# karfly/learnable-triangulation-pytorch

Measured on NVIDIA H100. Metric: volumetric samples/sec (4-view 384x384, 64^3 grid), higher is better.
Workload: dtype fp16x3 (split-fp16 operands, 3 wgmma products per term, fp32 accumulate)

## Files before the change

learnable-triangulation-pytorch_b200/csrc/conv_fold.cu:

```cuda
#include "tc_common.cuh"
#include "conv_tc_params.cuh"

namespace lt {

constexpr int kFoldThreads = 384;
constexpr int kFoldSmem = 227 * 1024;

template <int K>
struct FoldTile;
template <>
struct FoldTile<3> { static constexpr int BH = 8, BD = 2, KDS = 3; static constexpr bool RES = true; };
template <>
struct FoldTile<7> { static constexpr int BH = 16, BD = 2, KDS = 1; static constexpr bool RES = false; };

template <int K, int NC>
struct FoldCfg {
  static constexpr int BW = 8, BH = FoldTile<K>::BH, BD = FoldTile<K>::BD, KDS = FoldTile<K>::KDS;
  static constexpr bool RES = FoldTile<K>::RES;
  static constexpr int WBOX = BW + K - 1, HBOX = BH + K - 1, DBOX = BD + KDS - 1;
  static constexpr int A_BYTES = WBOX * HBOX * DBOX * 128;
  static constexpr int ASTAGES = K / KDS;
  static constexpr int TAP = NC * 128;
  static constexpr int B_SLICE = RES ? K * K * K * TAP : KDS * K * TAP;
  static constexpr int BLOCKS = BH * BD / 8;
  static constexpr int MB = RES ? BLOCKS : BLOCKS / 2;
  static constexpr int AVAIL = kFoldSmem - 1024 - 256;
  static constexpr int ARING_FIT = RES ? (AVAIL - B_SLICE) / A_BYTES : 2;
  static constexpr int ARING = ARING_FIT > 4 ? 4 : ARING_FIT;
  static constexpr int BRING_FIT = RES ? 1 : (AVAIL - ARING * A_BYTES) / B_SLICE;
  static constexpr int BRING = BRING_FIT > 4 ? 4 : BRING_FIT;
  static constexpr int A_OFF = BRING * B_SLICE;
  static constexpr int BAR_OFF = A_OFF + ARING * A_BYTES;
  static constexpr size_t SMEM = (size_t)BAR_OFF + 256 + 1024;
  static_assert(BW * BH * BD == (RES ? 128 : 256) && BH % 8 == 0 && MB == 2, "two m64 blocks of whole 8-wide lines per warpgroup");
  static_assert(A_BYTES % 1024 == 0 && B_SLICE % 1024 == 0, "boxes must start on 1024-byte swizzle atoms");
  static_assert(ARING >= 2 && BRING >= (RES ? 1 : 2) && 2 * (ARING + BRING) * 8 <= 256 && SMEM <= (size_t)kFoldSmem, "shared memory");
};

__device__ __forceinline__ void fold_tile_origin(const TcParams& p, int t, int& ow0, int& oh0, int& od0, int& nb) {
  ow0 = (t % p.tw) * p.bw; t /= p.tw;
  oh0 = (t % p.th) * p.bh; t /= p.th;
  od0 = (t % p.td) * p.bd;
  nb = t / p.td;
}

__device__ __forceinline__ void fold_load_line(uint32_t (&f)[2][4], uint32_t box, uint32_t row, uint32_t m) {
  const uint32_t a = box + row * 128u, sw = row & 7u;
  ldmatrix_x4(f[0], a + ((m ^ sw) << 4));
  ldmatrix_x4(f[1], a + (((m + 4u) ^ sw) << 4));
}

template <int NC>
__device__ __forceinline__ void fold_tap(float (&d1)[NC / 2], float (&d2)[NC / 2], const uint32_t (&l0)[2][4],
                                         const uint32_t (&l1)[2][4], uint64_t bd, uint32_t acc) {
  uint32_t a[4][4];
#pragma unroll
  for (int s = 0; s < 4; ++s) {
    const int q = s >> 1, c = 2 * (s & 1);
    a[s][0] = l0[q][c]; a[s][1] = l1[q][c]; a[s][2] = l0[q][c + 1]; a[s][3] = l1[q][c + 1];
  }
  wgmma_f16_rs<NC>(d1, a[0], bd, acc);
  wgmma_f16_rs<NC>(d1, a[1], bd + 2, 1u);
  wgmma_f16_rs<NC>(d2, a[0], bd + 4, acc);
  wgmma_f16_rs<NC>(d2, a[1], bd + 6, 1u);
  wgmma_f16_rs<NC>(d2, a[2], bd, 1u);
  wgmma_f16_rs<NC>(d2, a[3], bd + 2, 1u);
}

template <int K, int NC>
__global__ void __launch_bounds__(kFoldThreads, 1) conv_fold_kernel(const __grid_constant__ CUtensorMap tmA,
                                                                    const __grid_constant__ CUtensorMap tmB, const TcParams p) {
  using C = FoldCfg<K, NC>;
  extern __shared__ uint8_t smem_raw[];
  uint8_t* smem = reinterpret_cast<uint8_t*>((reinterpret_cast<uintptr_t>(smem_raw) + 1023) & ~(uintptr_t)1023);
  uint8_t* bsm = smem;
  uint8_t* asm_ = smem + C::A_OFF;
  uint64_t* afull = reinterpret_cast<uint64_t*>(smem + C::BAR_OFF);
  uint64_t* aempty = afull + C::ARING;
  uint64_t* bfull = aempty + C::ARING;
  uint64_t* bempty = bfull + C::BRING;

  const int wg = __shfl_sync(0xffffffffu, (int)(threadIdx.x >> 7), 0);
  const int lane = threadIdx.x & 31;
  const int ntiles = p.tw * p.th * p.td * p.tn;

  if (threadIdx.x == 0) {
    for (int s = 0; s < C::ARING; ++s) { mbar_init(&afull[s], 1); mbar_init(&aempty[s], C::RES ? 128 : 256); }
    for (int s = 0; s < C::BRING; ++s) { mbar_init(&bfull[s], 1); mbar_init(&bempty[s], 2); }
    fence_barrier_init();
    prefetch_tmap(&tmA);
    prefetch_tmap(&tmB);
  }
  __syncthreads();

  if (wg == 0) {
    regs_release_producer();
    if (threadIdx.x < 32) {
      if (C::RES && elect_one()) {
        mbar_expect_tx(&bfull[0], (uint32_t)C::B_SLICE);
        tma_load_3d(bsm, &tmB, &bfull[0], 0, 0, 0);
      }
      int sa = 0, sb = 0;
      uint32_t pa = 0, pb = 0;
      for (int t = blockIdx.x; t < ntiles; t += gridDim.x) {
        int ow0, oh0, od0, nb;
        fold_tile_origin(p, t, ow0, oh0, od0, nb);
        for (int as = 0; as < C::ASTAGES; ++as) {
          mbar_wait(&aempty[sa], pa ^ 1u);
          if (elect_one()) {
            mbar_expect_tx(&afull[sa], (uint32_t)C::A_BYTES);
            tma_load_5d(asm_ + (size_t)sa * C::A_BYTES, &tmA, &afull[sa], 0, ow0 - K / 2, oh0 - K / 2, od0 + as * C::KDS - K / 2, nb);
          }
          __syncwarp();
          if (++sa == C::ARING) { sa = 0; pa ^= 1u; }
          if constexpr (!C::RES) {
            for (int kw = 0; kw < K; ++kw) {
              mbar_wait(&bempty[sb], pb ^ 1u);
              if (elect_one()) {
                mbar_expect_tx(&bfull[sb], (uint32_t)C::B_SLICE);
                tma_load_3d(bsm + (size_t)sb * C::B_SLICE, &tmB, &bfull[sb], 0, 0, (kw * K + as * C::KDS) * K);
              }
              __syncwarp();
              if (++sb == C::BRING) { sb = 0; pb ^= 1u; }
            }
          }
        }
      }
    }
    return;
  }

  regs_claim_consumer();
  const int g = wg - 1, warp = (threadIdx.x >> 5) & 3;
  float d1[C::MB][NC / 2], d2[C::MB][NC / 2];
#pragma unroll
  for (int b = 0; b < C::MB; ++b)
#pragma unroll
    for (int i = 0; i < NC / 2; ++i) { d1[b][i] = 0.f; d2[b][i] = 0.f; }
  int blk_dd[C::MB], blk_hb[C::MB];
  uint32_t row0[C::MB];
#pragma unroll
  for (int b = 0; b < C::MB; ++b) {
    const int blk = C::RES ? b : C::MB * g + b;
    blk_dd[b] = blk / (C::BH / 8);
    blk_hb[b] = blk % (C::BH / 8);
    row0[b] = (uint32_t)((blk_dd[b] * C::HBOX + blk_hb[b] * 8 + 2 * warp) * C::WBOX + (lane & 7));
  }
  const uint32_t mlane = (uint32_t)(lane >> 3);
  const int r_lo = warp * 16 + (lane >> 2);
  const int c2 = 2 * (lane & 3);
  const uint32_t bsm0 = smem_u32(bsm), asm0 = smem_u32(asm_);
  const bool wg_lead = (threadIdx.x & 127) == 0;
  if (C::RES) mbar_wait(&bfull[0], 0);
  const int kt0 = C::RES ? g : 0, kstep = C::RES ? 2 : 1;
  int bprev = -1;
  for (int kt = kt0;; kt += kstep) {
    const int t = blockIdx.x + kt * gridDim.x;
    if (t >= ntiles) break;
#pragma unroll 1
    for (int as = 0; as < C::ASTAGES; ++as) {
      const int na = kt * C::ASTAGES + as;
      const int sa = na % C::ARING;
      mbar_wait(&afull[sa], (uint32_t)(na / C::ARING) & 1u);
      const uint32_t box = asm0 + (uint32_t)(sa * C::A_BYTES);
#pragma unroll 1
      for (int kw = 0; kw < K; ++kw) {
        const int nbs = na * K + kw;
        const int sb = C::RES ? 0 : nbs % C::BRING;
        if (!C::RES) mbar_wait(&bfull[sb], (uint32_t)(nbs / C::BRING) & 1u);
        const uint32_t bslice = bsm0 + (uint32_t)(sb * C::B_SLICE);
#pragma unroll
        for (int kdl = 0; kdl < C::KDS; ++kdl) {
          const int kd = as * C::KDS + kdl;
          const uint32_t roff = (uint32_t)(kdl * C::HBOX * C::WBOX + kw);
          uint32_t ln[K + 1][C::MB][2][4];
#pragma unroll
          for (int b = 0; b < C::MB; ++b) fold_load_line(ln[0][b], box, row0[b] + roff, mlane);
#pragma unroll
          for (int kh = 0; kh < K; ++kh) {
#pragma unroll
            for (int b = 0; b < C::MB; ++b) fold_load_line(ln[kh + 1][b], box, row0[b] + roff + (uint32_t)((kh + 1) * C::WBOX), mlane);
            wg_fence();
            const int tap = C::RES ? (kw * K + kd) * K + kh : kdl * K + kh;
            const uint64_t bd = make_sw128_desc(bslice + (uint32_t)(tap * C::TAP));
            const uint32_t acc = (as == 0 && kw == 0 && kdl == 0 && kh == 0) ? 0u : 1u;
#pragma unroll
            for (int b = 0; b < C::MB; ++b) fold_tap<NC>(d1[b], d2[b], ln[kh][b], ln[kh + 1][b], bd, acc);
            wg_commit();
            wg_wait<1>();
            if (!C::RES && kh == 0 && bprev >= 0) {
              if (wg_lead) mbar_arrive_local(&bempty[bprev]);
              bprev = -1;
            }
          }
        }
        if (!C::RES) bprev = sb;
      }
      mbar_arrive_local(&aempty[sa]);
    }
    wg_wait<0>();
    if (!C::RES) {
      if (wg_lead) mbar_arrive_local(&bempty[bprev]);
      bprev = -1;
    }
#pragma unroll
    for (int b = 0; b < C::MB; ++b) { wg_fence_regs(d1[b]); wg_fence_regs(d2[b]); }

    int ow0, oh0, od0, nb;
    fold_tile_origin(p, t, ow0, oh0, od0, nb);
#pragma unroll
    for (int b = 0; b < C::MB; ++b) {
#pragma unroll
      for (int h = 0; h < 2; ++h) {
        const int r = r_lo + 8 * h;
        const int ow = ow0 + (r & 7), oh = oh0 + blk_hb[b] * 8 + (r >> 3), od = od0 + blk_dd[b];
        if (!(ow < p.OW && oh < p.OH && od < p.OD)) continue;
        const long opix = (((long)nb * p.FD + od) * p.FH + oh) * p.FW + ow;
        conv_epilogue_row<NC>(p, d1[b], d2[b], h, opix, 0, c2);
        if constexpr (NC == 16) {
          const float z[8] = {0.f, 0.f, 0.f, 0.f, 0.f, 0.f, 0.f, 0.f};
          conv_epilogue_row<16>(p, z, z, h, opix, 16, c2);
        }
      }
    }
  }
}

template <int K, int NC>
static int launch_fold(const CUtensorMap& tmA, const CUtensorMap& tmB, const TcParams& p, cudaStream_t st) {
  using C = FoldCfg<K, NC>;
  static DeviceOnce configured;
  if (configured.first()) {
    cudaError_t e = cudaFuncSetAttribute(conv_fold_kernel<K, NC>, cudaFuncAttributeMaxDynamicSharedMemorySize, kFoldSmem);
    if (e != cudaSuccess) return fail(LT_ERR_CUDA, "conv_fold: cudaFuncSetAttribute: %s", cudaGetErrorString(e));
  }
  const long ntiles = (long)p.tw * p.th * p.td * p.tn;
  const int grid = (int)(ntiles < sm_count() ? ntiles : sm_count());
  conv_fold_kernel<K, NC><<<grid, kFoldThreads, C::SMEM, st>>>(tmA, tmB, p);
  cudaError_t e = cudaGetLastError();
  if (e != cudaSuccess) return fail(LT_ERR_CUDA, "conv_fold_kernel: %s", cudaGetErrorString(e));
  return LT_OK;
}

template <int K, int NC>
static int conv_fold_run(const lt_conv_desc* d, const void* in, const void* weight, const float* scale, const float* shift,
                         const void* residual, void* out, cudaStream_t st) {
  using C = FoldCfg<K, NC>;
  TcParams p;
  fill_params(d, p, 1, NC, NC, 3, scale, shift, residual, out);
  p.bw = C::BW; p.bh = C::BH; p.bd = C::BD; p.bn = 1;
  p.tw = ceil_div(d->OW, p.bw); p.th = ceil_div(d->OH, p.bh); p.td = ceil_div(d->OD, p.bd); p.tn = d->N;
  p.stages = C::ARING;
  CUtensorMap tmA, tmB;
  int rc = make_in_map(&tmA, d, C::WBOX, C::HBOX, C::DBOX, 1, in);
  if (rc) return rc;
  const uint64_t dims[3] = {64, (uint64_t)NC, (uint64_t)K * K * K};
  const uint64_t str[2] = {128, (uint64_t)NC * 128};
  const uint32_t bx[3] = {64, (uint32_t)NC, (uint32_t)(C::B_SLICE / C::TAP)};
  rc = make_map(&tmB, weight, 3, dims, str, bx, nullptr, 1);
  if (rc) return rc;
  return launch_fold<K, NC>(tmA, tmB, p, st);
}

int conv_fold_supported(const lt_conv_desc* d) {
  const bool cubic = d->KD == d->KH && d->KH == d->KW && (d->KW == 3 || d->KW == 7);
  const int pd = d->KW / 2;
  return cubic && d->Cin == 32 && d->Cout <= 32 && d->sd == 1 && d->sh == 1 && d->sw == 1 && d->pd == pd && d->ph == pd &&
         d->pw == pd && d->OD == d->ID && d->OH == d->IH && d->OW == d->IW && d->osd == 1 && d->osh == 1 && d->osw == 1 &&
         d->ood == 0 && d->ooh == 0 && d->oow == 0 && d->FD == d->OD && d->FH == d->OH && d->FW == d->OW && d->FC == 32 &&
         d->in_format == LT_FMT_S32 && d->IW >= 16;
}

int conv_fold_fwd(const lt_conv_desc* d, const void* in, const void* weight, const float* scale, const float* shift,
                  const void* residual, void* out, void* stream) {
  LT_REQUIRE(conv_fold_supported(d), "conv_fold: unsupported layer shape");
  const cudaStream_t st = (cudaStream_t)stream;
  const bool narrow = d->Cout <= 16;
  if (d->KW == 3)
    return narrow ? conv_fold_run<3, 16>(d, in, weight, scale, shift, residual, out, st)
                  : conv_fold_run<3, 32>(d, in, weight, scale, shift, residual, out, st);
  return narrow ? conv_fold_run<7, 16>(d, in, weight, scale, shift, residual, out, st)
                : conv_fold_run<7, 32>(d, in, weight, scale, shift, residual, out, st);
}

__global__ void __launch_bounds__(256) fold_pack_weights_kernel(const float* __restrict__ w, sh_t* __restrict__ out, int K, int Cout,
                                                                int NC) {
  const int total = K * K * K * NC * 32;
  for (int i = blockIdx.x * blockDim.x + threadIdx.x; i < total; i += gridDim.x * blockDim.x) {
    const int ci = i % 32;
    int r = i / 32;
    const int co = r % NC; r /= NC;
    const int kh = r % K; r /= K;
    const int kd = r % K;
    const int kw = r / K;
    const int tap = (kd * K + kh) * K + kw;
    const float v = co < Cout ? w[((long)tap * 32 + ci) * Cout + co] : 0.0f;
    sh_t hi, lo;
    split_s32(v, hi, lo);
    sh_t* rowp = out + ((long)((kw * K + kd) * K + kh) * NC + co) * 64;
    rowp[ci] = hi;
    rowp[32 + ci] = lo;
  }
}

}

using namespace lt;

extern "C" size_t lt_conv_fold_weight_bytes(int K, int Cout) {
  const int NC = (Cout + 15) & ~15;
  return (size_t)K * K * K * NC * 128;
}

extern "C" int lt_conv_fold_pack_weights(const float* w_tap_ci_co, void* packed, int K, int Cout, void* stream) {
  LT_REQUIRE(w_tap_ci_co && packed && (K == 3 || K == 7) && Cout > 0 && Cout <= 32, "conv_fold_pack_weights: bad arguments");
  const int NC = (Cout + 15) & ~15;
  const int total = K * K * K * NC * 32;
  fold_pack_weights_kernel<<<ceil_div(total, 256), 256, 0, (cudaStream_t)stream>>>(w_tap_ci_co, reinterpret_cast<sh_t*>(packed), K,
                                                                                   Cout, NC);
  LT_CHECK_LAUNCH("fold_pack_weights_kernel");
  return LT_OK;
}
```

learnable-triangulation-pytorch_b200/csrc/tc_common.cuh:

```cuda
#pragma once
#include "common.cuh"
#include <cuda.h>

namespace lt {

__device__ __forceinline__ uint32_t smem_u32(const void* p) { return (uint32_t)__cvta_generic_to_shared(p); }

__device__ __forceinline__ bool elect_one() {
  uint32_t pred;
  asm volatile("{\n\t.reg .pred p;\n\telect.sync _|p, 0xffffffff;\n\tselp.u32 %0, 1, 0, p;\n\t}" : "=r"(pred));
  return pred != 0;
}

__device__ __forceinline__ void mbar_init(uint64_t* bar, uint32_t count) {
  asm volatile("mbarrier.init.shared::cta.b64 [%0], %1;" ::"r"(smem_u32(bar)), "r"(count));
}
__device__ __forceinline__ void mbar_expect_tx(uint64_t* bar, uint32_t bytes) {
  asm volatile("mbarrier.arrive.expect_tx.shared::cta.b64 _, [%0], %1;" ::"r"(smem_u32(bar)), "r"(bytes) : "memory");
}
__device__ __forceinline__ bool mbar_try_wait(uint64_t* bar, uint32_t parity) {
  uint32_t ok;
  asm volatile(
      "{\n\t.reg .pred p;\n\t"
      "mbarrier.try_wait.parity.shared::cta.b64 p, [%1], %2;\n\t"
      "selp.u32 %0, 1, 0, p;\n\t}"
      : "=r"(ok)
      : "r"(smem_u32(bar)), "r"(parity)
      : "memory");
  return ok != 0;
}
__device__ __forceinline__ void mbar_wait(uint64_t* bar, uint32_t parity) {
  if (mbar_try_wait(bar, parity)) return;
  const long long t0 = clock64();
  while (!mbar_try_wait(bar, parity)) {
    if (clock64() - t0 > 4000000000LL) __trap();
  }
}
__device__ __forceinline__ void mbar_arrive_local(uint64_t* bar) {
  asm volatile("mbarrier.arrive.shared::cta.b64 _, [%0];" ::"r"(smem_u32(bar)) : "memory");
}
__device__ __forceinline__ void fence_barrier_init() { asm volatile("fence.mbarrier_init.release.cluster;" ::: "memory"); }
__device__ __forceinline__ void fence_proxy_async() { asm volatile("fence.proxy.async.shared::cta;" ::: "memory"); }

__device__ __forceinline__ void tma_load_5d(void* dst, const CUtensorMap* map, uint64_t* bar, int c0, int c1, int c2, int c3, int c4) {
  asm volatile(
      "cp.async.bulk.tensor.5d.shared::cluster.global.mbarrier::complete_tx::bytes [%0], [%1, {%3, %4, %5, %6, %7}], [%2];"
      ::"r"(smem_u32(dst)), "l"(map), "r"(smem_u32(bar)), "r"(c0), "r"(c1), "r"(c2), "r"(c3), "r"(c4)
      : "memory");
}
__device__ __forceinline__ void tma_load_3d(void* dst, const CUtensorMap* map, uint64_t* bar, int c0, int c1, int c2) {
  asm volatile(
      "cp.async.bulk.tensor.3d.shared::cluster.global.mbarrier::complete_tx::bytes [%0], [%1, {%3, %4, %5}], [%2];"
      ::"r"(smem_u32(dst)), "l"(map), "r"(smem_u32(bar)), "r"(c0), "r"(c1), "r"(c2)
      : "memory");
}
__device__ __forceinline__ void tma_load_2d(void* dst, const CUtensorMap* map, uint64_t* bar, int c0, int c1) {
  asm volatile(
      "cp.async.bulk.tensor.2d.shared::cluster.global.mbarrier::complete_tx::bytes [%0], [%1, {%3, %4}], [%2];"
      ::"r"(smem_u32(dst)), "l"(map), "r"(smem_u32(bar)), "r"(c0), "r"(c1)
      : "memory");
}
__device__ __forceinline__ void tma_store_5d(const CUtensorMap* map, const void* src, int c0, int c1, int c2, int c3, int c4) {
  asm volatile("cp.async.bulk.tensor.5d.global.shared::cta.bulk_group [%0, {%2, %3, %4, %5, %6}], [%1];"
               ::"l"(map), "r"(smem_u32(src)), "r"(c0), "r"(c1), "r"(c2), "r"(c3), "r"(c4)
               : "memory");
}
__device__ __forceinline__ void bulk_commit() { asm volatile("cp.async.bulk.commit_group;" ::: "memory"); }
__device__ __forceinline__ void bulk_wait_read0() { asm volatile("cp.async.bulk.wait_group.read 0;" ::: "memory"); }
__device__ __forceinline__ void bulk_wait0() { asm volatile("cp.async.bulk.wait_group 0;" ::: "memory"); }
__device__ __forceinline__ uint4 lds128(uint32_t a) {
  uint4 v;
  asm volatile("ld.shared.v4.u32 {%0, %1, %2, %3}, [%4];" : "=r"(v.x), "=r"(v.y), "=r"(v.z), "=r"(v.w) : "r"(a));
  return v;
}
__device__ __forceinline__ uint32_t lds32(uint32_t a) {
  uint32_t v;
  asm volatile("ld.shared.b32 %0, [%1];" : "=r"(v) : "r"(a));
  return v;
}
__device__ __forceinline__ void sts32(uint32_t a, uint32_t v) { asm volatile("st.shared.b32 [%0], %1;" ::"r"(a), "r"(v)); }
__device__ __forceinline__ float2 lds_f2(uint32_t a) {
  float2 v;
  asm volatile("ld.shared.v2.f32 {%0, %1}, [%2];" : "=f"(v.x), "=f"(v.y) : "r"(a));
  return v;
}
__device__ __forceinline__ void sts_f2(uint32_t a, float2 v) {
  asm volatile("st.shared.v2.f32 [%0], {%1, %2};" ::"r"(a), "f"(v.x), "f"(v.y));
}
__device__ __forceinline__ void prefetch_tmap(const CUtensorMap* map) {
  asm volatile("prefetch.tensormap [%0];" ::"l"(map) : "memory");
}

__device__ __forceinline__ void regs_release_producer() { asm volatile("setmaxnreg.dec.sync.aligned.u32 40;"); }
__device__ __forceinline__ void regs_claim_consumer() { asm volatile("setmaxnreg.inc.sync.aligned.u32 232;"); }

__device__ __forceinline__ void wg_fence() { asm volatile("wgmma.fence.sync.aligned;" ::: "memory"); }
__device__ __forceinline__ void wg_commit() { asm volatile("wgmma.commit_group.sync.aligned;" ::: "memory"); }
template <int N>
__device__ __forceinline__ void wg_wait() { asm volatile("wgmma.wait_group.sync.aligned %0;" ::"n"(N) : "memory"); }
template <int R>
__device__ __forceinline__ void wg_fence_regs(float (&d)[R]) {
#pragma unroll
  for (int i = 0; i < R; ++i) asm volatile("" : "+f"(d[i])::"memory");
}
template <int N>
__device__ __forceinline__ void wgmma_f16(float (&d)[N / 2], uint64_t ad, uint64_t bd, uint32_t scale_d);
template <>
__device__ __forceinline__ void wgmma_f16<16>(float (&d)[8], uint64_t ad, uint64_t bd, uint32_t scale_d) {
  asm volatile(
      "{\n\t.reg .pred p;\n\tsetp.ne.b32 p, %10, 0;\n\t"
      "wgmma.mma_async.sync.aligned.m64n16k16.f32.f16.f16 {%0,%1,%2,%3,%4,%5,%6,%7}, %8, %9, p, 1, 1, 0, 0;\n\t}"
      : "+f"(d[0]), "+f"(d[1]), "+f"(d[2]), "+f"(d[3]), "+f"(d[4]), "+f"(d[5]), "+f"(d[6]), "+f"(d[7])
      : "l"(ad), "l"(bd), "r"(scale_d));
}
template <>
__device__ __forceinline__ void wgmma_f16<32>(float (&d)[16], uint64_t ad, uint64_t bd, uint32_t scale_d) {
  asm volatile(
      "{\n\t.reg .pred p;\n\tsetp.ne.b32 p, %18, 0;\n\t"
      "wgmma.mma_async.sync.aligned.m64n32k16.f32.f16.f16 {%0,%1,%2,%3,%4,%5,%6,%7,%8,%9,%10,%11,%12,%13,%14,%15}, %16, %17, p, 1, 1, 0, 0;\n\t}"
      : "+f"(d[0]), "+f"(d[1]), "+f"(d[2]), "+f"(d[3]), "+f"(d[4]), "+f"(d[5]), "+f"(d[6]), "+f"(d[7]), "+f"(d[8]), "+f"(d[9]), "+f"(d[10]), "+f"(d[11]), "+f"(d[12]), "+f"(d[13]), "+f"(d[14]), "+f"(d[15])
      : "l"(ad), "l"(bd), "r"(scale_d));
}
template <>
__device__ __forceinline__ void wgmma_f16<64>(float (&d)[32], uint64_t ad, uint64_t bd, uint32_t scale_d) {
  asm volatile(
      "{\n\t.reg .pred p;\n\tsetp.ne.b32 p, %34, 0;\n\t"
      "wgmma.mma_async.sync.aligned.m64n64k16.f32.f16.f16 {%0,%1,%2,%3,%4,%5,%6,%7,%8,%9,%10,%11,%12,%13,%14,%15,%16,%17,%18,%19,%20,%21,%22,%23,%24,%25,%26,%27,%28,%29,%30,%31}, %32, %33, p, 1, 1, 0, 0;\n\t}"
      : "+f"(d[0]), "+f"(d[1]), "+f"(d[2]), "+f"(d[3]), "+f"(d[4]), "+f"(d[5]), "+f"(d[6]), "+f"(d[7]), "+f"(d[8]), "+f"(d[9]), "+f"(d[10]), "+f"(d[11]), "+f"(d[12]), "+f"(d[13]), "+f"(d[14]), "+f"(d[15]), "+f"(d[16]), "+f"(d[17]), "+f"(d[18]), "+f"(d[19]), "+f"(d[20]), "+f"(d[21]), "+f"(d[22]), "+f"(d[23]), "+f"(d[24]), "+f"(d[25]), "+f"(d[26]), "+f"(d[27]), "+f"(d[28]), "+f"(d[29]), "+f"(d[30]), "+f"(d[31])
      : "l"(ad), "l"(bd), "r"(scale_d));
}
template <>
__device__ __forceinline__ void wgmma_f16<128>(float (&d)[64], uint64_t ad, uint64_t bd, uint32_t scale_d) {
  asm volatile(
      "{\n\t.reg .pred p;\n\tsetp.ne.b32 p, %66, 0;\n\t"
      "wgmma.mma_async.sync.aligned.m64n128k16.f32.f16.f16 {%0,%1,%2,%3,%4,%5,%6,%7,%8,%9,%10,%11,%12,%13,%14,%15,%16,%17,%18,%19,%20,%21,%22,%23,%24,%25,%26,%27,%28,%29,%30,%31,%32,%33,%34,%35,%36,%37,%38,%39,%40,%41,%42,%43,%44,%45,%46,%47,%48,%49,%50,%51,%52,%53,%54,%55,%56,%57,%58,%59,%60,%61,%62,%63}, %64, %65, p, 1, 1, 0, 0;\n\t}"
      : "+f"(d[0]), "+f"(d[1]), "+f"(d[2]), "+f"(d[3]), "+f"(d[4]), "+f"(d[5]), "+f"(d[6]), "+f"(d[7]), "+f"(d[8]), "+f"(d[9]), "+f"(d[10]), "+f"(d[11]), "+f"(d[12]), "+f"(d[13]), "+f"(d[14]), "+f"(d[15]), "+f"(d[16]), "+f"(d[17]), "+f"(d[18]), "+f"(d[19]), "+f"(d[20]), "+f"(d[21]), "+f"(d[22]), "+f"(d[23]), "+f"(d[24]), "+f"(d[25]), "+f"(d[26]), "+f"(d[27]), "+f"(d[28]), "+f"(d[29]), "+f"(d[30]), "+f"(d[31]), "+f"(d[32]), "+f"(d[33]), "+f"(d[34]), "+f"(d[35]), "+f"(d[36]), "+f"(d[37]), "+f"(d[38]), "+f"(d[39]), "+f"(d[40]), "+f"(d[41]), "+f"(d[42]), "+f"(d[43]), "+f"(d[44]), "+f"(d[45]), "+f"(d[46]), "+f"(d[47]), "+f"(d[48]), "+f"(d[49]), "+f"(d[50]), "+f"(d[51]), "+f"(d[52]), "+f"(d[53]), "+f"(d[54]), "+f"(d[55]), "+f"(d[56]), "+f"(d[57]), "+f"(d[58]), "+f"(d[59]), "+f"(d[60]), "+f"(d[61]), "+f"(d[62]), "+f"(d[63])
      : "l"(ad), "l"(bd), "r"(scale_d));
}

template <int N>
__device__ __forceinline__ void wgmma_f16_rs(float (&d)[N / 2], const uint32_t (&a)[4], uint64_t bd, uint32_t scale_d);
template <>
__device__ __forceinline__ void wgmma_f16_rs<16>(float (&d)[8], const uint32_t (&a)[4], uint64_t bd, uint32_t scale_d) {
  asm volatile(
      "{\n\t.reg .pred p;\n\tsetp.ne.b32 p, %13, 0;\n\t"
      "wgmma.mma_async.sync.aligned.m64n16k16.f32.f16.f16 {%0,%1,%2,%3,%4,%5,%6,%7}, {%8,%9,%10,%11}, %12, p, 1, 1, 0;\n\t}"
      : "+f"(d[0]), "+f"(d[1]), "+f"(d[2]), "+f"(d[3]), "+f"(d[4]), "+f"(d[5]), "+f"(d[6]), "+f"(d[7])
      : "r"(a[0]), "r"(a[1]), "r"(a[2]), "r"(a[3]), "l"(bd), "r"(scale_d));
}
template <>
__device__ __forceinline__ void wgmma_f16_rs<32>(float (&d)[16], const uint32_t (&a)[4], uint64_t bd, uint32_t scale_d) {
  asm volatile(
      "{\n\t.reg .pred p;\n\tsetp.ne.b32 p, %21, 0;\n\t"
      "wgmma.mma_async.sync.aligned.m64n32k16.f32.f16.f16 {%0,%1,%2,%3,%4,%5,%6,%7,%8,%9,%10,%11,%12,%13,%14,%15}, {%16,%17,%18,%19}, %20, p, 1, 1, 0;\n\t}"
      : "+f"(d[0]), "+f"(d[1]), "+f"(d[2]), "+f"(d[3]), "+f"(d[4]), "+f"(d[5]), "+f"(d[6]), "+f"(d[7]), "+f"(d[8]), "+f"(d[9]), "+f"(d[10]), "+f"(d[11]), "+f"(d[12]), "+f"(d[13]), "+f"(d[14]), "+f"(d[15])
      : "r"(a[0]), "r"(a[1]), "r"(a[2]), "r"(a[3]), "l"(bd), "r"(scale_d));
}

__device__ __forceinline__ void ldmatrix_x4(uint32_t (&r)[4], uint32_t addr) {
  asm volatile("ldmatrix.sync.aligned.m8n8.x4.shared.b16 {%0, %1, %2, %3}, [%4];"
               : "=r"(r[0]), "=r"(r[1]), "=r"(r[2]), "=r"(r[3])
               : "r"(addr));
}

__device__ __forceinline__ void split_s32x2(float a, float b, uint32_t& hi2, uint32_t& lo2) {
  asm("cvt.rn.satfinite.f16x2.f32 %0, %1, %2;" : "=r"(hi2) : "f"(b), "f"(a));
  const float2 hf = __half22float2(*reinterpret_cast<const __half2*>(&hi2));
  const float ra = (a - hf.x) * kLoScale, rb = (b - hf.y) * kLoScale;
  asm("cvt.rn.satfinite.f16x2.f32 %0, %1, %2;" : "=r"(lo2) : "f"(rb), "f"(ra));
}

__device__ __forceinline__ uint64_t make_sw128_desc(uint32_t saddr) {
  return (uint64_t)((saddr & 0x3FFFFu) >> 4) | (1ull << 16) | ((uint64_t)(1024 >> 4) << 32) | (1ull << 62);
}

int make_map(CUtensorMap* map, const void* base, int rank, const uint64_t* dims, const uint64_t* strides_bytes,
             const uint32_t* box, const uint32_t* estrides, int swizzle128, int f32 = 0);

}
```

Baseline: 194.5.

## Merge hi/lo weight wgmmas into double-width N instructions with split-stacked weight layout

Reorders the weight slab so hi and lo fp16 halves are stacked along N (hi rows then lo rows, 64-byte swizzle), letting one wgmma with 2*NC columns compute both A_hi*B_hi and A_hi*B_lo at once. This cuts the per-tap wgmma count from six to four. A third accumulator holds the A_lo*B_hi term and is added into d2 in the epilogue. The cost is extra accumulator registers and a switch to a 64B swizzle TMA map and descriptor.

```diff
diff --git a/learnable-triangulation-pytorch_b200/csrc/conv_fold.cu b/learnable-triangulation-pytorch_b200/csrc/conv_fold.cu
--- a/learnable-triangulation-pytorch_b200/csrc/conv_fold.cu
+++ b/learnable-triangulation-pytorch_b200/csrc/conv_fold.cu
@@ -51,7 +51,7 @@
 }
 
 template <int NC>
-__device__ __forceinline__ void fold_tap(float (&d1)[NC / 2], float (&d2)[NC / 2], const uint32_t (&l0)[2][4],
+__device__ __forceinline__ void fold_tap(float (&d1)[NC / 2], float (&d2)[NC / 2], float (&d3)[NC / 2], const uint32_t (&l0)[2][4],
                                          const uint32_t (&l1)[2][4], uint64_t bd, uint32_t acc) {
   uint32_t a[4][4];
 #pragma unroll
@@ -59,12 +59,10 @@
     const int q = s >> 1, c = 2 * (s & 1);
     a[s][0] = l0[q][c]; a[s][1] = l1[q][c]; a[s][2] = l0[q][c + 1]; a[s][3] = l1[q][c + 1];
   }
-  wgmma_f16_rs<NC>(d1, a[0], bd, acc);
-  wgmma_f16_rs<NC>(d1, a[1], bd + 2, 1u);
-  wgmma_f16_rs<NC>(d2, a[0], bd + 4, acc);
-  wgmma_f16_rs<NC>(d2, a[1], bd + 6, 1u);
-  wgmma_f16_rs<NC>(d2, a[2], bd, 1u);
-  wgmma_f16_rs<NC>(d2, a[3], bd + 2, 1u);
+  wgmma_f16_rs_x2<2 * NC>(d1, d2, a[0], bd, acc);
+  wgmma_f16_rs_x2<2 * NC>(d1, d2, a[1], bd + 2, 1u);
+  wgmma_f16_rs<NC>(d3, a[2], bd, acc);
+  wgmma_f16_rs<NC>(d3, a[3], bd + 2, 1u);
 }
 
 template <int K, int NC>
@@ -132,11 +130,11 @@
 
   regs_claim_consumer();
   const int g = wg - 1, warp = (threadIdx.x >> 5) & 3;
-  float d1[C::MB][NC / 2], d2[C::MB][NC / 2];
+  float d1[C::MB][NC / 2], d2[C::MB][NC / 2], d3[C::MB][NC / 2];
 #pragma unroll
   for (int b = 0; b < C::MB; ++b)
 #pragma unroll
-    for (int i = 0; i < NC / 2; ++i) { d1[b][i] = 0.f; d2[b][i] = 0.f; }
+    for (int i = 0; i < NC / 2; ++i) { d1[b][i] = 0.f; d2[b][i] = 0.f; d3[b][i] = 0.f; }
   int blk_dd[C::MB], blk_hb[C::MB];
   uint32_t row0[C::MB];
 #pragma unroll
@@ -182,10 +180,10 @@
             for (int b = 0; b < C::MB; ++b) fold_load_line(ln[kh + 1][b], box, row0[b] + roff + (uint32_t)((kh + 1) * C::WBOX), mlane);
             wg_fence();
             const int tap = C::RES ? (kw * K + kd) * K + kh : kdl * K + kh;
-            const uint64_t bd = make_sw128_desc(bslice + (uint32_t)(tap * C::TAP));
+            const uint64_t bd = make_sw64_desc(bslice + (uint32_t)(tap * C::TAP));
             const uint32_t acc = (as == 0 && kw == 0 && kdl == 0 && kh == 0) ? 0u : 1u;
 #pragma unroll
-            for (int b = 0; b < C::MB; ++b) fold_tap<NC>(d1[b], d2[b], ln[kh][b], ln[kh + 1][b], bd, acc);
+            for (int b = 0; b < C::MB; ++b) fold_tap<NC>(d1[b], d2[b], d3[b], ln[kh][b], ln[kh + 1][b], bd, acc);
             wg_commit();
             wg_wait<1>();
             if (!C::RES && kh == 0 && bprev >= 0) {
@@ -204,7 +202,13 @@
       bprev = -1;
     }
 #pragma unroll
-    for (int b = 0; b < C::MB; ++b) { wg_fence_regs(d1[b]); wg_fence_regs(d2[b]); }
+    for (int b = 0; b < C::MB; ++b) {
+      wg_fence_regs(d1[b]);
+      wg_fence_regs(d2[b]);
+      wg_fence_regs(d3[b]);
+#pragma unroll
+      for (int i = 0; i < NC / 2; ++i) d2[b][i] += d3[b][i];
+    }
 
     int ow0, oh0, od0, nb;
     fold_tile_origin(p, t, ow0, oh0, od0, nb);
@@ -254,10 +258,10 @@
   CUtensorMap tmA, tmB;
   int rc = make_in_map(&tmA, d, C::WBOX, C::HBOX, C::DBOX, 1, in);
   if (rc) return rc;
-  const uint64_t dims[3] = {64, (uint64_t)NC, (uint64_t)K * K * K};
-  const uint64_t str[2] = {128, (uint64_t)NC * 128};
-  const uint32_t bx[3] = {64, (uint32_t)NC, (uint32_t)(C::B_SLICE / C::TAP)};
-  rc = make_map(&tmB, weight, 3, dims, str, bx, nullptr, 1);
+  const uint64_t dims[3] = {32, (uint64_t)(2 * NC), (uint64_t)K * K * K};
+  const uint64_t str[2] = {64, (uint64_t)NC * 128};
+  const uint32_t bx[3] = {32, (uint32_t)(2 * NC), (uint32_t)(C::B_SLICE / C::TAP)};
+  rc = make_map(&tmB, weight, 3, dims, str, bx, nullptr, 2);
   if (rc) return rc;
   return launch_fold<K, NC>(tmA, tmB, p, st);
 }
@@ -297,9 +301,9 @@
     const float v = co < Cout ? w[((long)tap * 32 + ci) * Cout + co] : 0.0f;
     sh_t hi, lo;
     split_s32(v, hi, lo);
-    sh_t* rowp = out + ((long)((kw * K + kd) * K + kh) * NC + co) * 64;
-    rowp[ci] = hi;
-    rowp[32 + ci] = lo;
+    sh_t* hrow = out + ((long)((kw * K + kd) * K + kh) * 2 * NC + co) * 32;
+    hrow[ci] = hi;
+    hrow[NC * 32 + ci] = lo;
   }
 }
 
diff --git a/learnable-triangulation-pytorch_b200/csrc/tc_common.cuh b/learnable-triangulation-pytorch_b200/csrc/tc_common.cuh
--- a/learnable-triangulation-pytorch_b200/csrc/tc_common.cuh
+++ b/learnable-triangulation-pytorch_b200/csrc/tc_common.cuh
@@ -157,6 +157,28 @@
       : "r"(a[0]), "r"(a[1]), "r"(a[2]), "r"(a[3]), "l"(bd), "r"(scale_d));
 }
 
+template <int N>
+__device__ __forceinline__ void wgmma_f16_rs_x2(float (&dl)[N / 4], float (&dh)[N / 4], const uint32_t (&a)[4], uint64_t bd,
+                                                uint32_t scale_d);
+template <>
+__device__ __forceinline__ void wgmma_f16_rs_x2<32>(float (&dl)[8], float (&dh)[8], const uint32_t (&a)[4], uint64_t bd,
+                                                    uint32_t scale_d) {
+  asm volatile(
+      "{\n\t.reg .pred p;\n\tsetp.ne.b32 p, %21, 0;\n\t"
+      "wgmma.mma_async.sync.aligned.m64n32k16.f32.f16.f16 {%0,%1,%2,%3,%4,%5,%6,%7,%8,%9,%10,%11,%12,%13,%14,%15}, {%16,%17,%18,%19}, %20, p, 1, 1, 0;\n\t}"
+      : "+f"(dl[0]), "+f"(dl[1]), "+f"(dl[2]), "+f"(dl[3]), "+f"(dl[4]), "+f"(dl[5]), "+f"(dl[6]), "+f"(dl[7]), "+f"(dh[0]), "+f"(dh[1]), "+f"(dh[2]), "+f"(dh[3]), "+f"(dh[4]), "+f"(dh[5]), "+f"(dh[6]), "+f"(dh[7])
+      : "r"(a[0]), "r"(a[1]), "r"(a[2]), "r"(a[3]), "l"(bd), "r"(scale_d));
+}
+template <>
+__device__ __forceinline__ void wgmma_f16_rs_x2<64>(float (&dl)[16], float (&dh)[16], const uint32_t (&a)[4], uint64_t bd,
+                                                    uint32_t scale_d) {
+  asm volatile(
+      "{\n\t.reg .pred p;\n\tsetp.ne.b32 p, %37, 0;\n\t"
+      "wgmma.mma_async.sync.aligned.m64n64k16.f32.f16.f16 {%0,%1,%2,%3,%4,%5,%6,%7,%8,%9,%10,%11,%12,%13,%14,%15,%16,%17,%18,%19,%20,%21,%22,%23,%24,%25,%26,%27,%28,%29,%30,%31}, {%32,%33,%34,%35}, %36, p, 1, 1, 0;\n\t}"
+      : "+f"(dl[0]), "+f"(dl[1]), "+f"(dl[2]), "+f"(dl[3]), "+f"(dl[4]), "+f"(dl[5]), "+f"(dl[6]), "+f"(dl[7]), "+f"(dl[8]), "+f"(dl[9]), "+f"(dl[10]), "+f"(dl[11]), "+f"(dl[12]), "+f"(dl[13]), "+f"(dl[14]), "+f"(dl[15]), "+f"(dh[0]), "+f"(dh[1]), "+f"(dh[2]), "+f"(dh[3]), "+f"(dh[4]), "+f"(dh[5]), "+f"(dh[6]), "+f"(dh[7]), "+f"(dh[8]), "+f"(dh[9]), "+f"(dh[10]), "+f"(dh[11]), "+f"(dh[12]), "+f"(dh[13]), "+f"(dh[14]), "+f"(dh[15])
+      : "r"(a[0]), "r"(a[1]), "r"(a[2]), "r"(a[3]), "l"(bd), "r"(scale_d));
+}
+
 __device__ __forceinline__ void ldmatrix_x4(uint32_t (&r)[4], uint32_t addr) {
   asm volatile("ldmatrix.sync.aligned.m8n8.x4.shared.b16 {%0, %1, %2, %3}, [%4];"
                : "=r"(r[0]), "=r"(r[1]), "=r"(r[2]), "=r"(r[3])
@@ -173,6 +195,9 @@
 __device__ __forceinline__ uint64_t make_sw128_desc(uint32_t saddr) {
   return (uint64_t)((saddr & 0x3FFFFu) >> 4) | (1ull << 16) | ((uint64_t)(1024 >> 4) << 32) | (1ull << 62);
 }
+__device__ __forceinline__ uint64_t make_sw64_desc(uint32_t saddr) {
+  return (uint64_t)((saddr & 0x3FFFFu) >> 4) | (1ull << 16) | ((uint64_t)(512 >> 4) << 32) | (2ull << 62);
+}
 
 int make_map(CUtensorMap* map, const void* base, int rank, const uint64_t* dims, const uint64_t* strides_bytes,
              const uint32_t* box, const uint32_t* estrides, int swizzle128, int f32 = 0);
```

Result: faster. 199.7, median of 6 (+2.7%).
